# DakeQQ/Automatic-Speech-Recognition-ASR-ONNX

Measured on AMD Instinct MI355X. Metric: audio-sec/s, SenseVoiceSmall, 8 s @ 16 kHz chunks, batch 64 per GPU (RTF = 1/value per GPU-stream), higher is better.
Workload: dtype bf16; 1 GPU; SenseVoiceSmall bf16 (234 M params, 70 SANM blocks), batch=64 x 8 s per GPU, greedy CTC; step k's audio is resident in HBM when the step starts, batch k+1's host->device copy (pinned, copy stream) and every token-id download are inside the timed region; global_batch=64, parallelism=dp1 (utterance sharding, RCCL arena broadcast + hypothesis gather)

## Files before the change

automatic-speech-recognition-asr-onnx_amd/csrc/kernels.h:

```cpp
#pragma once
#include "common.h"

struct UttPlan {
  int64_t audio_off;
  int32_t n_samples;
  int32_t n_frames;
  int32_t frame_off;
  int32_t n_lfr;
  int32_t T;
  int32_t row_off;
  int32_t lang;
  int32_t blk0;
};

enum { AUDIO_F32 = 0, AUDIO_I16 = 1, AUDIO_F16 = 2 };
inline size_t audio_elt_bytes(int audio_dtype) { return audio_dtype == AUDIO_F32 ? 4 : 2; }
struct FbankArgs {
  const void* audio;
  const UttPlan* plan;
  const int32_t* blk_utt;
  const int32_t* blk_f0;
  const float* dft_packed;
  const float* mel_packed;
  float* mel_out;
// ... 51 lines not shown
template <typename T>
void launch_decode_attention(const DecAttnArgs& a, int batch, hipStream_t s);
const char* decode_attn_last_kernel();

constexpr int BEAM_MAX = 8;
void launch_beam_topk(const float* logits, int ld, int rows, int n_valid, const float* bias, int K, float* topv, int32_t* topi, hipStream_t s);
struct BeamArgs {
  int beam, K, ld, first, n_slots;
  const float* topv; const int32_t* topi;
  float* cum; int32_t* fin; int32_t* len; int32_t* next; int32_t* done;
  const int32_t* stop; int n_stop;
  const int32_t *src_in, *tok_in; int32_t *src_out, *tok_out;
  const int32_t* slots_dev = nullptr;
  int slots_off = 0;
};
void launch_beam_select(const BeamArgs& a, int n_utt, hipStream_t s);

void launch_argmax_rows(const float* logits, int ld, int rows, int n_valid, const float* extra, int32_t* ids, hipStream_t s);
void launch_no_speech_prob(const float* logits, int ld, int rows, int n_valid, const float* penalty, int no_speech_id, float* prob, hipStream_t s);

void launch_apply_penalty(float* logits, int ld, int rows, const int32_t* save_ids, int ld_save, const int32_t* n_saved,
                          int range, float value, hipStream_t s, int partial = 0);
void launch_append_ids(const int32_t* next, int rows, int32_t* save_ids, int ld_save, const int32_t* n_saved, hipStream_t s);

struct SampleArgs {
  float* logits; int ld; int rows; int n_valid;
  const float* extra;
  const int32_t* save_ids; int ld_save; const int32_t* n_saved;
  float temperature, top_p, repetition_penalty; int top_k;
  const float* noise; uint64_t seed;
  int32_t* next;
};
void launch_sample_topk_topp(const SampleArgs& a, hipStream_t s);

struct LfrArgs {
  const float* mel;
  const UttPlan* plan;
  const int32_t* row_utt;
  const float* cmvn_means;
  const float* cmvn_vars;
  const float* speech_pos;
  const float* language_embed;
  const float* system_embed;
  float* out;
  int ld_out, feat, n_mels, lfr_m, lfr_n, n_prompt, n_rows;
  int affine_mode = 0;
  bf16_t* out_lo = nullptr;
};
void launch_lfr_cmvn(const LfrArgs& a, hipStream_t s);

template <typename OutT>
void launch_layernorm(const float* x, int ld_x, int rows, int D, const float* gamma, const float* beta, float eps,
                      OutT* out, int ld_out, int fill_to, hipStream_t s, const int32_t* rows_dev = nullptr);


struct AttnArgs {
  const void* q; const void* k; int ld_qk;
  int ld_q = 0;
  const void* vt; int ld_vt;
  void* ctx; int ld_ctx;
  const UttPlan* plan;
  const int32_t* qb_utt;
  const int32_t* qb_q0;
  int n_qblocks, n_heads;
  int qt = 0, n_waves = 4, max_T = 0;
  const UttPlan* q_plan = nullptr;
  int causal = 0, kv_group = 1;
};
void attention_geometry(int max_T, int head_dim, int* qt, int* n_waves);
void launch_attention_bf16_hd128(const AttnArgs& a, hipStream_t s);
void launch_attention_bf16_hd64(const AttnArgs& a, hipStream_t s);
void launch_attention_f32(const AttnArgs& a, int head_dim, hipStream_t s);

struct SanmFusedArgs {
  const void* h; int ld_h; int K;
  const void* wqkv; int ldw;
  const float* bqkv;
  const float* wfsmn; const float* bfsmn;
  const UttPlan* plan; int n_utts, n_heads, d;
  void* ctx; int ld_ctx;
  float* mem; int ld_mem;
  int n_rows_alloc;
  const float* ln_colsum = nullptr; int ln_dim = 0; float ln_eps = 1e-5f;
  const float2* ln_stats_in = nullptr; int ln_slots = 0;
  int dbg = 0;
};
bool sanm_fused_supported(int max_T, int d_head, int n_heads, int d, int fsmn_taps, int K);

struct SanmBlockLayer {
  const float *bqkv, *cqkv, *wfsmn, *bfsmn, *b1, *c1, *b2;
  const void* wpack;
};
struct SanmBlockArgs {
  const bf16_t* wqkv; const float* bqkv; const float* cqkv;
  const float* wfsmn; const float* bfsmn;
  const bf16_t* wout;
  const bf16_t* w1; const float* b1; const float* c1;
  const bf16_t* w2; const float* b2;
  const SanmBlockLayer* layers = nullptr; int n_layers = 1;
  int flag_stride = 0;
  unsigned* place = nullptr;
  int times_layer = 0;
  int st_in_n = 16;
  int opt = 0;
  int ffnk = 0;
  const void* wpack = nullptr;
// ... 144 lines not shown
```

automatic-speech-recognition-asr-onnx_amd/csrc/kernels.hip:

```cpp
#include "kernels.h"
#include "gemm.h"

#include <algorithm>
#include <type_traits>
#include <cstdlib>

namespace {

constexpr int HOP = 160, WIN = 400;
constexpr int FB_FRAMES = 64;
constexpr int FB_SPAN = (FB_FRAMES - 1) * HOP + WIN;
constexpr int FB_AUDIO_LDS = FB_SPAN + FB_SPAN / HOP + 16;
constexpr int FB_PLD = 273;

template <typename S> struct Pcm;
template <> struct Pcm<float> {
  typedef float raw_t;
  static __device__ __forceinline__ raw_t load(const float* p, int i) { return p[i]; }
  static __device__ __forceinline__ raw_t hold(raw_t r) { return r; }
  static __device__ __forceinline__ float widen(raw_t r, float) { return r; }
};
template <> struct Pcm<int16_t> {
  typedef int raw_t;
  static __device__ __forceinline__ raw_t load(const int16_t* p, int i) { return p[i]; }
// ... 293 lines not shown
    const int k = kc * 32 + fgrp * 8 + e;
    float v = 0.0f;
    if (k < n_kchunks16 * 16) {
      v = dft_packed[(((size_t)tr * n_kchunks16 + (k >> 4)) * 64 + ((k & 3) * 16 + frow)) * 4 + ((k & 15) >> 2)];
    }
    float r = v;
    for (int z = 0; z < 3; ++z) {
      const uint32_t b = pack_bf16x2(r, 0.0f) & 0xffffu;
      r -= __uint_as_float(b << 16);
      w[z][e >> 1] |= b << ((e & 1) * 16);
    }
  }
  for (int z = 0; z < 3; ++z) out[((size_t)(tr * FB_K32 + kc) * 3 + z) * 64 + lane] = make_uint4(w[z][0], w[z][1], w[z][2], w[z][3]);
}

__global__ void lfr_cmvn_kernel(const LfrArgs a) {
  const int m = blockIdx.x;
  float* o = a.out + (size_t)m * a.ld_out;
  const int u = a.row_utt[m];
  bf16_t* olo = a.out_lo ? a.out_lo + (size_t)m * a.ld_out : nullptr;
  if (u < 0) {
    for (int c = threadIdx.x; c < a.ld_out; c += blockDim.x) { o[c] = 0.0f; if (olo) olo[c] = 0; }
    return;
  }
  const UttPlan up = a.plan[u];
  const int t = m - up.row_off;
  const int left = (a.lfr_m - 1) / 2;
  for (int c = threadIdx.x; c < a.ld_out; c += blockDim.x) {
    float v = 0.0f;
    if (c < a.feat && t < up.T) {
      if (a.n_prompt > 0 && t == 0) {
        v = a.language_embed[(size_t)up.lang * a.feat + c];
      } else if (t < a.n_prompt) {
        v = a.system_embed[(size_t)(t - 1) * a.feat + c];
      } else {
        const int j = t - a.n_prompt;
        int f = j * a.lfr_n + c / a.n_mels - left;
        f = min(max(f, 0), up.n_frames - 1);
        const float x = a.mel[(size_t)(up.frame_off + f) * a.n_mels + c % a.n_mels];
        if (a.affine_mode == 1) {
          v = x * a.cmvn_vars[c] + a.speech_pos[(size_t)j * a.feat + c];
        } else {
          v = (x + a.cmvn_means[c]) * a.cmvn_vars[c];
          v = v + a.speech_pos[(size_t)j * a.feat + c];
        }
      }
    }
    o[c] = v;
    if (olo) olo[c] = f32_to_bf16(v);
  }
}

constexpr int LN_MAXV = 8;
template <typename OutT>
__global__ __launch_bounds__(256) void layernorm_kernel(const float* __restrict__ x, int ld_x, int rows, int D,
                                                        const float* __restrict__ gamma, const float* __restrict__ beta,
                                                        float eps, OutT* out, int ld_out, int fill_to, const int32_t* __restrict__ rows_dev) {
  const int row = blockIdx.x * 4 + (threadIdx.x >> 6);
  const int lane = threadIdx.x & 63;
  if (row >= rows || (rows_dev && row >= *rows_dev)) return;
  const float* xr = x + (size_t)row * ld_x;
  float4 v[LN_MAXV];
  float s = 0.0f;
#pragma unroll
  for (int k = 0; k < LN_MAXV; ++k) {
    const int i = k * 256 + lane * 4;
    v[k] = (i < D) ? *reinterpret_cast<const float4*>(xr + i) : make_float4(0.f, 0.f, 0.f, 0.f);
    s += (v[k].x + v[k].y) + (v[k].z + v[k].w);
  }
  const float mean = wave_sum(s) / (float)D;
  float q = 0.0f;
#pragma unroll
  for (int k = 0; k < LN_MAXV; ++k) {
    const int i = k * 256 + lane * 4;
    if (i < D) {
      const float a = v[k].x - mean, b = v[k].y - mean, c = v[k].z - mean, d = v[k].w - mean;
      q += (a * a + b * b) + (c * c + d * d);
    }
  }
  const float var = wave_sum(q) / (float)D;
  const float rstd = 1.0f / sqrtf(var + eps);
  OutT* o = out + (size_t)row * ld_out;
#pragma unroll
  for (int k = 0; k < LN_MAXV; ++k) {
    const int i = k * 256 + lane * 4;
    if (i < D) {
      float y0 = (v[k].x - mean) * rstd, y1 = (v[k].y - mean) * rstd, y2 = (v[k].z - mean) * rstd, y3 = (v[k].w - mean) * rstd;
      if (gamma) {
        const float4 g = *reinterpret_cast<const float4*>(gamma + i);
        const float4 b = *reinterpret_cast<const float4*>(beta + i);
        y0 = y0 * g.x + b.x; y1 = y1 * g.y + b.y; y2 = y2 * g.z + b.z; y3 = y3 * g.w + b.w;
      }
      if constexpr (sizeof(OutT) == 4) {
        *reinterpret_cast<float4*>(o + i) = make_float4(y0, y1, y2, y3);
      } else {
        uint2 w;
        w.x = pack_bf16x2(y0, y1);
        w.y = pack_bf16x2(y2, y3);
        *reinterpret_cast<uint2*>(o + i) = w;
      }
    }
  }
  for (int i = D + lane; i < fill_to; i += 64) Elem<OutT>::store(o + i, 0.0f);
}

__global__ __launch_bounds__(256) void layernorm_fp8_kernel(const float* __restrict__ x, int ld_x, int rows, int D, float eps, float inv_scale,
                                                            unsigned char* __restrict__ out, int ld_out) {
  const int row = blockIdx.x * 4 + (threadIdx.x >> 6), lane = threadIdx.x & 63;
  if (row >= rows) return;
  const float* xr = x + (size_t)row * ld_x;
  float4 v[8];
  const int nv = D >> 8;
  float s1 = 0.0f;
#pragma unroll
  for (int k = 0; k < 8; ++k)
    if (k < nv) { v[k] = *reinterpret_cast<const float4*>(xr + k * 256 + lane * 4); s1 += (v[k].x + v[k].y) + (v[k].z + v[k].w); }
  const float mean = wave_sum(s1) / (float)D;
  float s2 = 0.0f;
#pragma unroll
  for (int k = 0; k < 8; ++k)
    if (k < nv) { const float a = v[k].x - mean, b = v[k].y - mean, c = v[k].z - mean, d = v[k].w - mean; s2 += (a * a + b * b) + (c * c + d * d); }
  const float rstd = rsqrtf(wave_sum(s2) / (float)D + eps) * inv_scale;
#pragma unroll
  for (int k = 0; k < 8; ++k)
    if (k < nv) {
      auto q = [&](float t) { return fminf(fmaxf((t - mean) * rstd, -448.0f), 448.0f); };
      int w = 0;
      w = __builtin_amdgcn_cvt_pk_fp8_f32(q(v[k].x), q(v[k].y), w, false);
      w = __builtin_amdgcn_cvt_pk_fp8_f32(q(v[k].z), q(v[k].w), w, true);
      *reinterpret_cast<int*>(out + (size_t)row * ld_out + k * 256 + lane * 4) = w;
    }
}

__device__ __forceinline__ float vmax3(float a, float b, float c) { return fmaxf(fmaxf(a, b), c); }

template <int HD, int CHUNK, int QT>
__global__ __launch_bounds__(512, (HD * QT <= 128) ? 4 : (HD * QT <= 256 ? 2 : 1)) void attn_bf16_kernel(const AttnArgs a, int n_rows_alloc) {
  constexpr int SLOTS = HD / 8;
  constexpr int KROWB = HD * 2;
  constexpr int K_RPI = 64 / SLOTS;
  constexpr int VSLOTS = CHUNK / 8;
  constexpr int VROWB = CHUNK * 2;
  constexpr int V_RPI = 64 / VSLOTS;
  constexpr int V_NI = HD / V_RPI;
  static_assert(VSLOTS == 16 || VSLOTS == 32, "V^T swizzle assumes 16 or 32 slots per row");
  extern __shared__ __attribute__((aligned(16))) unsigned char smem[];
  unsigned char* Ks = smem;
  unsigned char* Vs = smem + CHUNK * KROWB;

  const int tid = threadIdx.x, lane = tid & 63;
  const int wave = __builtin_amdgcn_readfirstlane(tid >> 6), NW = blockDim.x >> 6;
  const int fq = lane & 15, g = lane >> 4;
  const int u = a.qb_utt[blockIdx.x], q_base = a.qb_q0[blockIdx.x], h = blockIdx.y;
// ... 926 lines not shown
  ASR_REQUIRE(a.n_kchunks * 16 == WIN, "fbank: k-chunks must cover the window");
  const size_t lds = (size_t)(FB_AUDIO_LDS + FB_FRAMES * FB_PLD) * sizeof(float);
  static PerDeviceOnce attr_once;
  if (attr_once.first()) {
    HIP_CHECK(hipFuncSetAttribute(reinterpret_cast<const void*>(fbank_kernel<S>), hipFuncAttributeMaxDynamicSharedMemorySize, (int)lds));
  }
  if (a.dft_split) {
    FbankArgs b = a;
    if (const char* e = getenv("ASR_FBANK_DBG")) b.dbg = atoi(e);
    const size_t lds2 = (size_t)FB_A16 * 2 * 2 + (size_t)FB_FRAMES * FB_PLD * sizeof(float);
    static PerDeviceOnce attr2_once;
    if (attr2_once.first()) {
      HIP_CHECK(hipFuncSetAttribute(reinterpret_cast<const void*>(fbank_split_kernel<S>), hipFuncAttributeMaxDynamicSharedMemorySize, (int)lds2));
    }
    hipLaunchKernelGGL(fbank_split_kernel<S>, dim3(n_blocks), dim3(64 * FB_WAVES), lds2, s, b);
    HIP_CHECK(hipGetLastError());
    return;
  }
  hipLaunchKernelGGL(fbank_kernel<S>, dim3(n_blocks), dim3(256), lds, s, a);
  HIP_CHECK(hipGetLastError());
}
void launch_fbank(const FbankArgs& a, int n_blocks, hipStream_t s) {
  switch (a.audio_dtype) {
    case AUDIO_F32: return launch_fbank_typed<float>(a, n_blocks, s);
    case AUDIO_I16: return launch_fbank_typed<int16_t>(a, n_blocks, s);
    case AUDIO_F16: return launch_fbank_typed<_Float16>(a, n_blocks, s);
    default: ASR_THROW(ASR_ERR_INVALID, "fbank: unknown audio sample type %d", a.audio_dtype);
  }
}

size_t fbank_split_table_bytes(int n_bin_tiles, int win) {
  ASR_REQUIRE(win == WIN, "fbank: only win=400 is built (got %d)", win);
  return (size_t)n_bin_tiles * 2 * FB_K32 * 3 * 64 * 16;
}
void launch_fbank_split_table(const float* dft_packed, int n_bin_tiles, int n_kchunks16, void* out, hipStream_t s) {
  const int total = n_bin_tiles * 2 * FB_K32 * 64;
  hipLaunchKernelGGL(fbank_split_table_kernel, dim3((total + 255) / 256), dim3(256), 0, s, dft_packed, n_bin_tiles, n_kchunks16, reinterpret_cast<uint4*>(out));
  HIP_CHECK(hipGetLastError());
}

void launch_lfr_cmvn(const LfrArgs& a, hipStream_t s) {
  hipLaunchKernelGGL(lfr_cmvn_kernel, dim3(a.n_rows), dim3(256), 0, s, a);
  HIP_CHECK(hipGetLastError());
}

template <typename OutT>
void launch_layernorm(const float* x, int ld_x, int rows, int D, const float* gamma, const float* beta, float eps,
                      OutT* out, int ld_out, int fill_to, hipStream_t s, const int32_t* rows_dev) {
  ASR_REQUIRE(D % 4 == 0 && D <= LN_MAXV * 256 && ld_x % 4 == 0 && ld_out % 4 == 0, "layernorm: D=%d ld=%d unsupported", D, ld_x);
  hipLaunchKernelGGL(layernorm_kernel<OutT>, dim3((rows + 3) / 4), dim3(256), 0, s, x, ld_x, rows, D, gamma, beta, eps, out,
                     ld_out, fill_to, rows_dev);
  HIP_CHECK(hipGetLastError());
}
template void launch_layernorm<float>(const float*, int, int, int, const float*, const float*, float, float*, int, int, hipStream_t, const int32_t*);
template void launch_layernorm<bf16_t>(const float*, int, int, int, const float*, const float*, float, bf16_t*, int, int, hipStream_t, const int32_t*);

void launch_layernorm_fp8(const float* x, int ld_x, int rows, int D, float eps, float inv_scale, unsigned char* out, int ld_out, hipStream_t s) {
  ASR_REQUIRE(D % 256 == 0 && D <= 2048 && ld_x % 4 == 0 && ld_out % 4 == 0, "layernorm_fp8: D=%d unsupported", D);
  hipLaunchKernelGGL(layernorm_fp8_kernel, dim3((rows + 3) / 4), dim3(256), 0, s, x, ld_x, rows, D, eps, inv_scale, out, ld_out);
  HIP_CHECK(hipGetLastError());
}

template <int HD, int CHUNK, int QT>
static void launch_attn_inst(const AttnArgs& a, hipStream_t s) {
  constexpr int lds = CHUNK * HD * 2 * 2;
  static PerDeviceOnce attr_once;
  if (attr_once.first()) {
    HIP_CHECK(hipFuncSetAttribute(reinterpret_cast<const void*>(attn_bf16_kernel<HD, CHUNK, QT>),
                                  hipFuncAttributeMaxDynamicSharedMemorySize, lds));
  }
  AttnArgs b = a;
  if (b.ld_q == 0) b.ld_q = b.ld_qk;
  hipLaunchKernelGGL((attn_bf16_kernel<HD, CHUNK, QT>), dim3(a.n_qblocks, a.n_heads), dim3(64 * a.n_waves), lds, s, b, a.ld_vt);
  HIP_CHECK(hipGetLastError());
}

void attention_geometry(int max_T, int head_dim, int* qt, int* nw) {
  const int qt_max = 2;
  const int n_tiles = (max_T + 15) / 16;
  int q = 1;
  while (q < qt_max && (n_tiles + q - 1) / q > 8) ++q;
  if (const char* e = getenv("ASR_ATTN_QT")) q = std::max(1, std::min(qt_max, atoi(e)));
  int w = std::min(8, (n_tiles + q - 1) / q);
  if (const char* e = getenv("ASR_ATTN_NW")) w = std::max(1, std::min(8, atoi(e)));
  *qt = q;
  *nw = w;
}

void launch_attention_bf16_hd128(const AttnArgs& a, hipStream_t s) {
  ASR_REQUIRE(a.qt >= 1 && a.qt <= 2 && a.n_waves >= 1 && a.n_waves <= 8, "attention: bad geometry qt=%d nw=%d", a.qt, a.n_waves);
  const bool big = a.max_T <= 256;
  if (a.qt == 1) { big ? launch_attn_inst<128, 256, 1>(a, s) : launch_attn_inst<128, 128, 1>(a, s); }
  else { big ? launch_attn_inst<128, 256, 2>(a, s) : launch_attn_inst<128, 128, 2>(a, s); }
}
void launch_attention_bf16_hd64(const AttnArgs& a, hipStream_t s) {
  ASR_REQUIRE(a.qt >= 1 && a.qt <= 2 && a.n_waves >= 1 && a.n_waves <= 8, "attention: bad geometry qt=%d nw=%d", a.qt, a.n_waves);
  if (a.qt == 1) launch_attn_inst<64, 256, 1>(a, s); else launch_attn_inst<64, 256, 2>(a, s);
}

void launch_attention_f32(const AttnArgs& a, int head_dim, hipStream_t s) {
  ASR_REQUIRE(head_dim <= 128 && head_dim % 4 == 0, "attention_f32: head_dim %d unsupported", head_dim);
  AttnArgs b = a;
  if (b.ld_q == 0) b.ld_q = b.ld_qk;
  const int wgs = a.n_qblocks * a.n_heads;
  const int z = wgs >= 1024 ? 1 : wgs >= 256 ? 4 : 16;
  hipLaunchKernelGGL(attn_f32_kernel, dim3(a.n_qblocks, a.n_heads, z), dim3(256), 0, s, b, head_dim);
// ... 1078 lines not shown
```

automatic-speech-recognition-asr-onnx_amd/csrc/sanm_block8.hip:

```cpp
#include <algorithm>
#include <type_traits>
#include <utility>
#include "kernels.h"

namespace {

constexpr int R = 144, RF = 9;
constexpr int HD = 128, NH = 4, D = 512, DFF = 2048;
constexpr int NW = 8, NT = NW * 64;
constexpr int TAPS = 11;
constexpr int LDS_BYTES = 160 * 1024;
constexpr int CH = R * 256;
constexpr int NSLOT = 4;
constexpr int QS = 0, KS = CH, KEYS = 160, VS = KS + KEYS * 256, IMG_END = VS + HD * 512;
constexpr int TERM = CH;
constexpr int RED = 2 * CH;
constexpr int ST_F = NSLOT * CH;
constexpr int ST_P = ST_F + R * 8;
constexpr int DUMMY = ST_P + NSLOT * R * 8;
static_assert(IMG_END <= ST_F && TERM + R * HD * 4 <= ST_F && DUMMY + NW * 256 <= LDS_BYTES, "LDS map");

constexpr size_t PK_QKV = 0, PK_QKV_WAVE = 16 * 3 * 1024;
constexpr size_t PK_OUT = PK_QKV + (size_t)NH * NW * PK_QKV_WAVE, PK_OUT_WAVE = 8 * 2 * 1024;
constexpr size_t PK_W1 = PK_OUT + (size_t)NH * NW * PK_OUT_WAVE, PK_W1_WAVE = 16 * 4 * 1024;
constexpr size_t PK_W2 = PK_W1 + (size_t)NH * NW * PK_W1_WAVE, PK_W2_WAVE = 32 * 2 * 1024;
constexpr size_t PK_BYTES = PK_W2 + (size_t)NH * NW * PK_W2_WAVE;
static_assert(PK_BYTES == (size_t)(3 * D * D + D * D + 2 * DFF * D) * 2, "the packed copy holds every weight element once");

__device__ __host__ constexpr int frag_col(int j, int fr) { return (j >> 1) * 32 + ((fr >> 2) << 3) + ((j & 1) << 2) + (fr & 3); }
template <int N> __device__ __forceinline__ void wait_vm() { asm volatile("s_waitcnt vmcnt(%0)" ::"n"(N) : "memory"); }

typedef __attribute__((ext_vector_type(4))) unsigned int u32x4_t;
__device__ __forceinline__ void store16_wt(void* p, uint4 v, bool plain = false) {
  if (plain) { *reinterpret_cast<uint4*>(p) = v; return; }
  const u32x4_t w = {v.x, v.y, v.z, v.w};
  asm volatile("global_store_dwordx4 %0, %1, off sc1\n\ts_nop 1" ::"v"(p), "v"(w) : "memory");
}
__device__ __forceinline__ void store8_wt(void* p, float2 v, bool plain = false) {
  if (plain) { *reinterpret_cast<float2*>(p) = v; return; }
  const f32x2_t w = {v.x, v.y};
  asm volatile("global_store_dwordx2 %0, %1, off sc1\n\ts_nop 1" ::"v"(p), "v"(w) : "memory");
}

__device__ __forceinline__ void publish(unsigned* flag, bool withhold = false) {
  wait_vm<0>();
  __syncthreads();
  if (threadIdx.x == 0 && !withhold) __hip_atomic_fetch_add(flag, 1u, __ATOMIC_RELAXED, __HIP_MEMORY_SCOPE_AGENT);
}
__device__ __forceinline__ void consume(unsigned* flag, unsigned need, unsigned* err, bool fence = true) {
  if (threadIdx.x == 0) {
    unsigned spins = 0;
    while (__hip_atomic_load(flag, __ATOMIC_RELAXED, __HIP_MEMORY_SCOPE_AGENT) < need) {
      __builtin_amdgcn_s_sleep(2);
      if (++spins > (1u << 15)) { __hip_atomic_store(err, 1u, __ATOMIC_RELAXED, __HIP_MEMORY_SCOPE_AGENT); break; }
      if ((spins & 255u) == 0u && __hip_atomic_load(err, __ATOMIC_RELAXED, __HIP_MEMORY_SCOPE_AGENT)) break;
    }
    if (fence) __builtin_amdgcn_fence(__ATOMIC_ACQUIRE, "agent");
  }
  __syncthreads();
}

__device__ __forceinline__ uint4 pack8(const float (&v)[8]) {
  uint4 w;
  w.x = pack_bf16x2(v[0], v[1]); w.y = pack_bf16x2(v[2], v[3]); w.z = pack_bf16x2(v[4], v[5]); w.w = pack_bf16x2(v[6], v[7]);
  return w;
}
__device__ __forceinline__ void stats8(const uint4& w, float& s1, float& s2) {
  const uint32_t wd[4] = {w.x, w.y, w.z, w.w};
#pragma unroll
  for (int e = 0; e < 4; ++e) {
    const float lo = __uint_as_float(wd[e] << 16), hi = __uint_as_float(wd[e] & 0xffff0000u);
    s1 += lo + hi;
    s2 = fmaf(lo, lo, fmaf(hi, hi, s2));
// ... 347 lines not shown
          const float2 ss = sum_row_partials(a->st_in + (size_t)(row0 + min(tid, rows_left - 1)) * (D / 32), D / 32);
          const float mean = ss.x * (1.0f / D);
          const float var = fmaxf(ss.y * (1.0f / D) - mean * mean, 0.0f);
          st_fin[tid] = make_float2(mean, rsqrtf(var + a->ln_eps));
        }
        __syncthreads();
      } else row_stats_from_chunks(smem, h, a->ln_eps, tid);
      STAMP_A(4);
      {
        unsigned char* dst = smem + (grp == 0 ? QS : KS);
        const float b8[8] = {b0.x, b0.y, b0.z, b0.w, b1.x, b1.y, b1.z, b1.w}, c8[8] = {c0.x, c0.y, c0.z, c0.w, c1.x, c1.y, c1.z, c1.w};
#pragma unroll
        for (int i = 0; i < RF; ++i) {
          const int row = i * 16 + frow;
          const float2 mr = st_fin[row];
          float v[8];
#pragma unroll
          for (int r = 0; r < 4; ++r) { v[r] = acc[i][0][r]; v[4 + r] = acc[i][1][r]; }
#pragma unroll
          for (int e = 0; e < 8; ++e) v[e] = (v[e] - mr.x * c8[e]) * mr.y + b8[e];
          *reinterpret_cast<uint4*>(dst + row * 256 + ((((col >> 3)) ^ (row & 15)) << 4)) = pack8(v);
        }
        unsigned char* vdst = smem + VS + dcol * 512 + (fgrp & 1) * 8;
#pragma unroll
        for (int i = 0; i < RF; ++i) {
          float v[4] = {acc[i][2][0], acc[i][2][1], acc[i][2][2], acc[i][2][3]};
#pragma unroll
          for (int r = 0; r < 4; ++r) { const float2 mr = st_fin[i * 16 + fgrp * 4 + r]; v[r] = (v[r] - mr.x * cs) * mr.y + bv; }
          uint2 w;
          w.x = pack_bf16x2(v[0], v[1]);
          w.y = pack_bf16x2(v[2], v[3]);
          *reinterpret_cast<uint2*>(vdst + (((2 * i + (fgrp >> 1)) ^ (dcol & 15)) << 4)) = w;
        }
        if (tid < 2 * HD) {
          const int d = tid & (HD - 1), slot = 18 + (tid >> 7);
          *reinterpret_cast<uint4*>(smem + VS + d * 512 + ((slot ^ (d & 15)) << 4)) = make_uint4(0, 0, 0, 0);
        }
      }
    }
    __syncthreads();
    STAMP_A(5);
    float wc[TAPS];
#pragma unroll
    for (int j = 0; j < TAPS; ++j) wc[j] = L->wfsmn[(h * HD + (tid & (HD - 1))) * TAPS + j];
    const float bc = L->bfsmn[h * HD + (tid & (HD - 1))];

    {
      const unsigned char* Qs = smem + QS;
      const unsigned char* Ks = smem + KS;
      const unsigned char* Vs = smem + VS;
      const int fq = frow, g = fgrp;
      const int n_sub = (T + 31) >> 5;
      const bool shared_tile = T > 128;
      auto scores = [&](const bf16x8_t (&qf)[HD / 32], bf16x8_t (&pf)[5], float& inv) {
        constexpr float LOG2E = 1.4426950408889634f;
        f32x4_t st[5][2];
#pragma unroll
        for (int s = 0; s < 5; ++s) { st[s][0] = f32x4_t{0.f, 0.f, 0.f, 0.f}; st[s][1] = f32x4_t{0.f, 0.f, 0.f, 0.f}; }
#pragma unroll
        for (int s = 0; s < 5; ++s) {
          if (s < n_sub) {
            const int key0 = s * 32 + ((fq >> 2) << 3) + (fq & 3), key1 = key0 + 4;
#pragma unroll
            for (int ks = 0; ks < HD / 32; ++ks) {
              const int c = ks * 4 + g;
              const bf16x8_t kf0 = *reinterpret_cast<const bf16x8_t*>(Ks + key0 * 256 + ((c ^ (key0 & 15)) << 4));
              const bf16x8_t kf1 = *reinterpret_cast<const bf16x8_t*>(Ks + key1 * 256 + ((c ^ (key1 & 15)) << 4));
              st[s][0] = __builtin_amdgcn_mfma_f32_16x16x32_bf16(kf0, qf[ks], st[s][0], 0, 0, 0);
              st[s][1] = __builtin_amdgcn_mfma_f32_16x16x32_bf16(kf1, qf[ks], st[s][1], 0, 0, 0);
            }
          }
        }
        float mx = -INFINITY;
#pragma unroll
        for (int s = 0; s < 5; ++s) {
          if (s * 32 + 32 > T) {
#pragma unroll
            for (int hlf = 0; hlf < 2; ++hlf)
#pragma unroll
              for (int r = 0; r < 4; ++r)
                if (s * 32 + g * 8 + hlf * 4 + r >= T) st[s][hlf][r] = -INFINITY;
          }
          mx = fmaxf(fmaxf(fmaxf(mx, fmaxf(st[s][0][0], st[s][0][1])), fmaxf(st[s][0][2], st[s][0][3])), fmaxf(fmaxf(st[s][1][0], st[s][1][1]), fmaxf(st[s][1][2], st[s][1][3])));
        }
        mx = fmaxf(mx, __shfl_xor(mx, 16, 64));
        mx = fmaxf(mx, __shfl_xor(mx, 32, 64));
        const f32x2_t mneg = {-mx * LOG2E, -mx * LOG2E}, l2 = {LOG2E, LOG2E};
        f32x2_t lsum = {0.0f, 0.0f};
#pragma unroll
        for (int s = 0; s < 5; ++s) {
          f32x2_t p[4];
#pragma unroll
          for (int q = 0; q < 4; ++q) {
            const f32x2_t e = __builtin_elementwise_fma(f32x2_t{st[s][q >> 1][2 * (q & 1)], st[s][q >> 1][2 * (q & 1) + 1]}, l2, mneg);
            p[q] = f32x2_t{__builtin_amdgcn_exp2f(e[0]), __builtin_amdgcn_exp2f(e[1])};
          }
          lsum += (p[0] + p[1]) + (p[2] + p[3]);
          union { bf16x8_t v; uint32_t w[4]; } u8;
#pragma unroll
          for (int q = 0; q < 4; ++q) u8.w[q] = pack_bf16x2(p[q][0], p[q][1]);
          pf[s] = u8.v;
        }
        float l = lsum[0] + lsum[1];
        l += __shfl_xor(l, 16, 64);
        l += __shfl_xor(l, 32, 64);
        inv = 1.0f / l;
      };
      auto context = [&](const bf16x8_t (&pf)[5], float inv, int qrow, auto dt0_tag, auto nd_tag) {
        constexpr int ND = decltype(nd_tag)::value;
        const int dt0 = dt0_tag;
        f32x4_t ot[ND];
#pragma unroll
        for (int e = 0; e < ND; ++e) ot[e] = f32x4_t{0.f, 0.f, 0.f, 0.f};
#pragma unroll
        for (int s = 0; s < 5; ++s) {
          if (s < n_sub) {
#pragma unroll
            for (int e = 0; e < ND; ++e) {
              const int d = (dt0 + e) * 16 + fq;
              const bf16x8_t vf = *reinterpret_cast<const bf16x8_t*>(Vs + d * 512 + (((s * 4 + g) ^ (d & 15)) << 4));
              ot[e] = __builtin_amdgcn_mfma_f32_16x16x32_bf16(vf, pf[s], ot[e], 0, 0, 0);
            }
          }
        }
        unsigned char* crow = smem + QS + qrow * 256;
#pragma unroll
        for (int e = 0; e < ND; ++e) {
          uint2 w;
          w.x = pack_bf16x2(ot[e][0] * inv, ot[e][1] * inv);
          w.y = pack_bf16x2(ot[e][2] * inv, ot[e][3] * inv);
          *reinterpret_cast<uint2*>(crow + ((((dt0 + e) * 2 + (g >> 1)) ^ (qrow & 15)) << 4) + (g & 1) * 8) = w;
        }
      };
      if (wave * 16 < T) {
        const int qrow = wave * 16 + fq;
        bf16x8_t qf[HD / 32], pf[5];
#pragma unroll
        for (int ks = 0; ks < HD / 32; ++ks) qf[ks] = *reinterpret_cast<const bf16x8_t*>(Qs + qrow * 256 + (((ks * 4 + g) ^ (qrow & 15)) << 4));
        float inv;
        scores(qf, pf, inv);
        context(pf, inv, qrow, 0, std::integral_constant<int, HD / 16>{});
      }
      STAMP_A(6);
      if (shared_tile) {
        bf16x8_t qf8[HD / 32], pf[5];
        const int qrow8 = 128 + fq;
#pragma unroll
        for (int ks = 0; ks < HD / 32; ++ks) qf8[ks] = *reinterpret_cast<const bf16x8_t*>(Qs + qrow8 * 256 + (((ks * 4 + g) ^ (qrow8 & 15)) << 4));
        float inv;
        scores(qf8, pf, inv);
        __syncthreads();
        context(pf, inv, 128 + fq, wave, std::integral_constant<int, 1>{});
      }
      STAMP_A(7);
    }
    __syncthreads();
    STAMP(2);
    {
      const bool plain = cluster_plain_stores(place, a->opt);
      if (a->times && tid == 0) a->times[(size_t)blockIdx.x * 16 + 15] = plain ? 1ull : 0ull;
      const int T16 = n_act * 16;
      for (int c = T * 16 + tid; c < T16 * 16; c += NT) *reinterpret_cast<uint4*>(smem + QS + c * 16) = make_uint4(0, 0, 0, 0);
      __syncthreads();
      store_chunk_img(reinterpret_cast<unsigned char*>(a->ctx + (size_t)row0 * D) + (size_t)h * T16 * 256, smem + QS, n_act * 4, wave, lane, plain);
    }
    STAMP(3);
#pragma unroll
    for (int i = 0; i < RF; ++i) {
      if (kh == 0) {
        const float* xr = a->x + (size_t)(row0 + min(i * 16 + frow, rows_left - 1)) * D + h * HD + cg * 32 + fgrp * 8;
        accb[i][0] = *reinterpret_cast<const f32x4_t*>(xr); accb[i][1] = *reinterpret_cast<const f32x4_t*>(xr + 4);
      } else { accb[i][0] = f32x4_t{0.f, 0.f, 0.f, 0.f}; accb[i][1] = f32x4_t{0.f, 0.f, 0.f, 0.f}; }
    }
    {
      constexpr int PAD = (TAPS - 1) / 2;
      const int c = tid & (HD - 1), seg = tid >> 7;
      const int t0 = seg < 2 ? seg * 40 : 80 + (seg - 2) * 32, len = seg < 2 ? 40 : 32;
      const unsigned char* vrow = smem + VS + c * 512;
      float x[56];
#pragma unroll
      for (int q = 0; q < 7; ++q) {
        const int sl = (t0 >> 3) - 1 + q;
        if (sl < 0 || sl * 8 >= T) {
#pragma unroll
          for (int e = 0; e < 8; ++e) x[q * 8 + e] = 0.0f;
        } else {
          const uint4 raw = *reinterpret_cast<const uint4*>(vrow + ((sl ^ (c & 15)) << 4));
          const uint32_t wds[4] = {raw.x, raw.y, raw.z, raw.w};
#pragma unroll
          for (int e = 0; e < 4; ++e) {
            x[q * 8 + 2 * e] = (sl * 8 + 2 * e < T) ? __uint_as_float(wds[e] << 16) : 0.0f;
            x[q * 8 + 2 * e + 1] = (sl * 8 + 2 * e + 1 < T) ? __uint_as_float(wds[e] & 0xffff0000u) : 0.0f;
          }
        }
      }
      float y[40];
#pragma unroll
      for (int i = 0; i < 40; ++i) {
        float accv = bc;
#pragma unroll
        for (int j = 0; j < TAPS; ++j) accv = fmaf(wc[j], x[8 + i + j - PAD], accv);
        y[i] = accv;
      }
// ... 419 lines not shown
```

automatic-speech-recognition-asr-onnx_amd/csrc/sensevoice.hip:

```cpp
#include <cstdlib>
#include <cstring>
#include <type_traits>

#include "../../include/asr_mi355x.h"
#include "engine.h"
#include "gemm.h"
#include "kernels.h"

namespace {

struct SvBlock {
  const float *ln1_g, *ln1_b, *bqkv, *wfsmn, *bfsmn, *ln2_g, *ln2_b, *b1, *b2;
  const float *cqkv, *c1;
  const void *wqkv, *wout, *w1, *w2;
  int in_size, kpad;
};

inline int round_up(int v, int m) { return (v + m - 1) / m * m; }

struct SvRunCtx;

struct PfDecLayer {
  const void *w1, *w2, *wq, *wkv, *wo;
  const float *b1, *b2, *n2_g, *n2_b, *wfsmn, *bq, *bkv, *bo;
// ... 327 lines not shown
  const bool tiles = r.tiles && block_cooldown == 0 && !foreign_now;
  HIP_CHECK(hipMemsetAsync(d_flags.ptr, 0, (tile_flag0 + (tiles ? (size_t)c.n_blocks * tile_flag_stride : 0)) * 4, stream));
  const float* x_in = d_x0.as<float>();
  const bf16_t* x_in_lo = x0lo;
  const float2* st_in = nullptr;
  bool st_in_block8 = false;
  float2* sta = d_sta.as<float2>();
  float2* stb = d_stb.as<float2>();
  int ld_in = kpad0;
  float* xa = d_xa.as<float>();
  float* xb = d_xb.as<float>();
  T* h = d_h.as<T>();
  T* qk = d_qk.as<T>();
  T* vt = d_vt.as<T>();
  T* ctx = d_ctx.as<T>();
  float* mem = d_mem.as<float>();
  T* ffn = d_ffn.as<T>();
  for (int i = 0; i < c.n_blocks; ++i) {
    const SvBlock& b = blocks[i];
    if constexpr (sizeof(T) == 2) {
      if (blk && b.in_size == d && x_in == xa) {
        if (!alg && i == 1) {
          ProfScope ps0(prof, "layernorm", stream);
          launch_rows_to_bf16(xa, xalo, (size_t)Mpad * d, stream);
          st_in = nullptr;
        }
        const int per = sanm_block_max_utts();
        const int run_end = (!paraformer && i < c.n_main) ? c.n_main : c.n_blocks;
        const int n_run = block_persist ? run_end - i : 1;
        for (int u0 = 0; u0 < r.batch; u0 += per) {
          ProfScope ps(prof, "sanm_block", stream);
          SanmBlockArgs ba{};
          ba.wqkv = (const bf16_t*)b.wqkv; ba.bqkv = b.bqkv; ba.cqkv = b.cqkv; ba.wfsmn = b.wfsmn; ba.bfsmn = b.bfsmn;
          ba.wout = (const bf16_t*)b.wout; ba.w1 = (const bf16_t*)b.w1; ba.b1 = b.b1; ba.c1 = b.c1; ba.w2 = (const bf16_t*)b.w2; ba.b2 = b.b2;
          ba.x_lo = xalo; ba.st_in = st_in; ba.x = xa; ba.x_lo_out = xalo; ba.st_out = sta;
          ba.ctx = (bf16_t*)ctx; ba.x1_lo = xblo; ba.st1 = stb; ba.hid = (bf16_t*)ffn;
          ba.plan = r.dp; ba.utt0 = u0; ba.n_utts = std::min(per, r.batch - u0);
          ba.flags = d_flags.as<unsigned>() + ((size_t)i * r.batch + u0) * 4; ba.err = d_flags.as<unsigned>() + flag_words;
          ba.flag_stride = r.batch * 4; ba.place = d_flags.as<unsigned>() + flag_words + 4 + (size_t)i * r.batch + u0;
          ba.n_rows_alloc = Mpad; ba.ln_eps = 1e-5f; ba.scatter = block_scatter; ba.fault = (block_fault && i == 1) ? 1 : 0;
          if (block_dbg >= i && block_dbg < i + n_run && u0 == 0) {
            d_times.reserve(256 * 16 * 8, stream); HIP_CHECK(hipMemsetAsync(d_times.ptr, 0, 256 * 16 * 8, stream)); ba.times = d_times.as<unsigned long long>();
            ba.times_layer = block_dbg - i;
          }
          ba.layers = d_layer_tab.as<SanmBlockLayer>() + i; ba.n_layers = n_run; ba.opt = block8_opt; ba.ffnk = block_ffnk ? 1 : 0;
          ba.st_in_n = st_in_block8 ? 4 : 16;
          launch_sanm_block8(ba, stream);
        }
        i += n_run - 1;
        st_in = sta;
        st_in_block8 = true;
        if (i == c.n_main - 1 && !paraformer) {
          ProfScope ps2(prof, "layernorm", stream);
          launch_layernorm<bf16_t>(xa, d, rows, d, after_g, after_b, 1e-5f, xalo, d, d, stream); st_in = nullptr;
          launch_layernorm<float>(xa, d, rows, d, after_g, after_b, 1e-5f, xa, d, d, stream);
        }
        continue;
      }
    }
    if constexpr (sizeof(T) == 2) {
      if (tiles && !blk && b.in_size == d && x_in == xa) {
        const int run_end = (!paraformer && i < c.n_main) ? c.n_main : c.n_blocks;
        {
          ProfScope ps(prof, "sanm_tiles", stream);
          SanmTilesArgs ta;
          ta.plan = r.dp; ta.tile_win = r.d_tile_win; ta.tile_idx = r.d_tile_idx; ta.n_tiles = r.n_tiles; ta.n_windows = r.batch; ta.n_layers = run_end - i;
          ta.ln_eps = 1e-5f; ta.layers = d_tlayer_tab.as<StreamLayer>() + i;
          ta.x = xa; ta.xb = xb; ta.ctx = (bf16_t*)ctx; ta.hid = (bf16_t*)ffn; ta.kv = d_tkv.as<bf16_t>(); ta.kv_parity_stride = (size_t)Mpad * 2 * d;
          ta.flags = d_flags.as<unsigned>() + tile_flag0 + (size_t)i * tile_flag_stride; ta.flag_stride = (int)tile_flag_stride;
          ta.err = d_flags.as<unsigned>() + flag_words; ta.opt = tiles_opt;
          if (tiles_dbg >= i && tiles_dbg < run_end) {
            d_times.reserve(256 * 16 * 8, stream); HIP_CHECK(hipMemsetAsync(d_times.ptr, 0, 256 * 16 * 8, stream)); ta.times = d_times.as<unsigned long long>();
            ta.times_layer = tiles_dbg - i;
          }
          launch_sanm_tiles(ta, stream);
        }
        i = run_end - 1;
        st_in = nullptr;
        if (i == c.n_main - 1 && !paraformer) {
          ProfScope ps2(prof, "layernorm", stream);
          launch_layernorm<float>(xa, d, rows, d, after_g, after_b, 1e-5f, xa, d, d, stream);
        }
        continue;
      }
    }
    if (!alg) {
      ProfScope ps(prof, "layernorm", stream);
      launch_layernorm<T>(x_in, ld_in, rows, b.in_size, b.ln1_g, b.ln1_b, 1e-5f, h, b.kpad, b.kpad, stream);
    }
    const bool fused = use_fused && precision == ASR_PRECISION_BF16 &&
                       sanm_fused_supported(r.max_T, c.d_head, c.n_heads, d, c.fsmn_kernel, b.kpad);
    if (fused) {
      ProfScope ps(prof, "sanm_fused", stream);
      SanmFusedArgs fa;
      fa.h = h; fa.ld_h = b.kpad; fa.K = b.kpad;
      if (alg) { fa.h = x_in_lo; fa.ln_colsum = b.cqkv; fa.ln_dim = b.in_size; fa.ln_stats_in = st_in; fa.ln_slots = d / 32; } fa.wqkv = b.wqkv; fa.ldw = b.kpad; fa.bqkv = b.bqkv;
      fa.wfsmn = b.wfsmn; fa.bfsmn = b.bfsmn; fa.plan = r.dp; fa.n_utts = r.batch; fa.n_heads = c.n_heads; fa.d = d;
      fa.ctx = ctx; fa.ld_ctx = d; fa.mem = mem; fa.ld_mem = d; fa.n_rows_alloc = Mpad;
      launch_sanm_qkv_attn(fa, stream);
    } else {
      {
        ProfScope ps(prof, "gemm_qkv", stream);
        GemmArgs g;
        g.A = h; g.lda = b.kpad; g.W = b.wqkv; g.ldw = b.kpad; g.M = rows; g.N = 2 * d; g.K = b.kpad; g.bias = b.bqkv;
        g.out_lo = qk; g.ld_out_lo = 2 * d;
        gemm(g);
        GemmArgs gv;
        gv.A = h; gv.lda = b.kpad; gv.W = (const T*)b.wqkv + (size_t)2 * d * b.kpad; gv.ldw = b.kpad; gv.M = rows; gv.N = d;
// ... 1 lines not shown
        gemm(gv);
      }
      {
        ProfScope ps(prof, "fsmn", stream);
        launch_fsmn<T>(vt, Mpad, b.wfsmn, b.bfsmn, d, c.fsmn_kernel, r.dp, r.d_row_utt, Mpad, mem, d, stream);
      }
      {
        ProfScope ps(prof, "attention", stream);
        AttnArgs aa;
        aa.q = qk; aa.k = qk + d; aa.ld_qk = 2 * d; aa.vt = vt; aa.ld_vt = Mpad; aa.ctx = ctx; aa.ld_ctx = d;
        aa.plan = r.dp; aa.qb_utt = r.d_qb_utt; aa.qb_q0 = r.d_qb_q0; aa.n_qblocks = r.n_qb; aa.n_heads = c.n_heads;
        aa.qt = r.att_qt; aa.n_waves = r.att_nw; aa.max_T = r.max_T;
        if (precision == ASR_PRECISION_BF16) launch_attention_bf16_hd128(aa, stream);
        else launch_attention_f32(aa, c.d_head, stream);
      }
    }
    {
      ProfScope ps(prof, "gemm_out", stream);
      GemmArgs g;
      g.A = ctx; g.lda = d; g.W = b.wout; g.ldw = d; g.M = rows; g.N = d; g.K = d;
      g.add = mem; g.ld_add = d;
      if (b.in_size == d) { g.add2 = x_in; g.ld_add2 = ld_in; }
      g.out_f32 = xb; g.ld_out_f32 = d;
      if (alg) { g.out_lo = xblo; g.ld_out_lo = d; g.st_out = stb; }
      gemm(g);
    }
    if (!alg) {
      ProfScope ps(prof, "layernorm", stream);
      launch_layernorm<T>(xb, d, rows, d, b.ln2_g, b.ln2_b, 1e-5f, h, d, d, stream);
    }
    {
      ProfScope ps(prof, "gemm_ffn1", stream);
      GemmArgs g;
      g.A = h; g.lda = d; g.W = b.w1; g.ldw = d; g.M = rows; g.N = dff; g.K = d; g.bias = b.b1; g.act = ACT_RELU;
      g.out_lo = ffn; g.ld_out_lo = dff;
      if (alg) { g.A = xblo; g.ln_colsum = b.c1; g.ln_dim = d; g.ln_stats_in = stb; g.ln_slots = d / 32; }
      gemm(g);
    }
    {
      ProfScope ps(prof, "gemm_ffn2", stream);
      GemmArgs g;
      g.A = ffn; g.lda = dff; g.W = b.w2; g.ldw = dff; g.M = rows; g.N = d; g.K = dff; g.bias = b.b2;
      g.add = xb; g.ld_add = d; g.out_f32 = xa; g.ld_out_f32 = d;
      if (alg) { g.out_lo = xalo; g.ld_out_lo = d; g.st_out = sta; }
      gemm(g);
    }
    x_in = xa;
    x_in_lo = xalo;
    st_in = sta;
    ld_in = d;
    if (i == 0) save_tap("block0", xa, rows, d, d, 4);
    if (i == c.n_main - 1 && !paraformer) {
      ProfScope ps(prof, "layernorm", stream);
      if (alg) { launch_layernorm<bf16_t>(xa, d, rows, d, after_g, after_b, 1e-5f, xalo, d, d, stream); st_in = nullptr; }
      launch_layernorm<float>(xa, d, rows, d, after_g, after_b, 1e-5f, xa, d, d, stream);
    }
  }
  if (paraformer) { copy_block_status(r); enqueue_paraformer_tail<T>(r); return; }
  if (taps_enabled) {
    launch_layernorm<float>(xa, d, rows, d, tp_g, tp_b, 1e-5f, xb, d, d, stream);
    save_tap("enc_out", xb, rows, d, d, 4);
  }
  {
    ProfScope ps(prof, "layernorm", stream);
    launch_layernorm<T>(xa, d, rows, d, tp_g, tp_b, 1e-5f, h, d, d, stream);
  }
  {
    ProfScope ps(prof, "gemm_ctc", stream);
    GemmArgs g;
    g.A = h; g.lda = d; g.W = ctc_w; g.ldw = d; g.M = rows; g.N = vpad; g.K = d; g.bias = ctc_b;
    g.amax_val = d_amax_v.as<float>(); g.amax_idx = d_amax_i.as<int32_t>(); g.n_valid = c.vocab;
    if (taps_enabled) { g.out_f32 = d_logits.as<float>(); g.ld_out_f32 = vpad; }
    gemm(g);
  }
  {
    ProfScope ps(prof, "ctc_tail", stream);
    launch_argmax_reduce(d_amax_v.as<float>(), d_amax_i.as<int32_t>(), rows, n_slabs, d_ids.as<int32_t>(), stream);
    launch_ctc_collapse(d_ids.as<int32_t>(), r.dp, r.batch, c.blank_id, d_tok.as<int32_t>(), r.max_tokens, d_num.as<int32_t>(), stream);
  }
  if (taps_enabled) {
    save_tap("logits", d_logits.ptr, rows, c.vocab, vpad, 4);
    save_tap("frame_ids", d_ids.ptr, rows, 1, 1, 4);
  }
  HIP_CHECK(hipMemcpyAsync(h_out.ptr, d_tok.ptr, (size_t)r.batch * r.max_tokens * 4, hipMemcpyDeviceToHost, stream));
  HIP_CHECK(hipMemcpyAsync(h_out.as<unsigned char>() + (size_t)r.batch * r.max_tokens * 4, d_num.ptr, (size_t)r.batch * 4,
                           hipMemcpyDeviceToHost, stream));
  copy_block_status(r);
}


template <typename T>
void SvSession::enqueue_paraformer_tail(const SvRunCtx& r) {
  const auto& c = cfg;
  const int d = c.d_model, dd = pcfg.d_dec_ffn, rows = r.rows, Mpad = r.Mpad, n_slabs = vpad / 64;
  float* xa = d_xa.as<float>();
  float* enc32 = d_xb.as<float>();
  T* enc_lo = d_enc_lo.as<T>();
  T* h = d_h.as<T>();
  T* q = d_qk.as<T>();
  T* ck = d_ck.as<T>();
  T* cvt = d_vt.as<T>();
  T* ctx = d_ctx.as<T>();
  T* ffn = d_ffn.as<T>();
  float* ffn32 = d_ffn32.as<float>();
  float* x1 = d_mem.as<float>();
  float* dec = d_dec.as<float>();
  float* x2 = d_x2.as<float>();
  float* x2_own = d_sa.as<float>();
// ... 985 lines not shown
```

Measured before the change: 79020 audio-s/s.

## Compute ninth query tile scores once across waves and fuse dual layernorm

In the SANM block8 attention path, when T exceeds 128 the ninth 16-row query tile was scored redundantly by every wave. Now waves 0-4 each compute one key sub-tile of those scores, reusing the K fragments already loaded for their own rows. They hand the partial maxima, probabilities and row sums over through new LDS regions with two extra barriers, so the other waves no longer repeat the full score pass. Separately, the post-encoder layernorm writes bf16 and fp32 outputs from one kernel instead of two launches. This removes a re-read of the activations and one launch, though the kernel now writes its fp32 result in place over its own input.

```diff
diff --git a/automatic-speech-recognition-asr-onnx_amd/csrc/kernels.h b/automatic-speech-recognition-asr-onnx_amd/csrc/kernels.h
--- a/automatic-speech-recognition-asr-onnx_amd/csrc/kernels.h
+++ b/automatic-speech-recognition-asr-onnx_amd/csrc/kernels.h
@@ -127,6 +127,7 @@
 template <typename OutT>
 void launch_layernorm(const float* x, int ld_x, int rows, int D, const float* gamma, const float* beta, float eps,
                       OutT* out, int ld_out, int fill_to, hipStream_t s, const int32_t* rows_dev = nullptr);
+void launch_layernorm_dual(const float* x, int ld_x, int rows, int D, const float* gamma, const float* beta, float eps, bf16_t* out_lo, float* out_f, int ld_out, hipStream_t s);
 
 
 struct AttnArgs {
diff --git a/automatic-speech-recognition-asr-onnx_amd/csrc/kernels.hip b/automatic-speech-recognition-asr-onnx_amd/csrc/kernels.hip
--- a/automatic-speech-recognition-asr-onnx_amd/csrc/kernels.hip
+++ b/automatic-speech-recognition-asr-onnx_amd/csrc/kernels.hip
@@ -369,10 +369,10 @@
 }
 
 constexpr int LN_MAXV = 8;
-template <typename OutT>
+template <typename OutT, bool DUAL = false>
 __global__ __launch_bounds__(256) void layernorm_kernel(const float* __restrict__ x, int ld_x, int rows, int D,
                                                         const float* __restrict__ gamma, const float* __restrict__ beta,
-                                                        float eps, OutT* out, int ld_out, int fill_to, const int32_t* __restrict__ rows_dev) {
+                                                        float eps, OutT* out, int ld_out, int fill_to, const int32_t* __restrict__ rows_dev, float* out_f = nullptr) {
   const int row = blockIdx.x * 4 + (threadIdx.x >> 6);
   const int lane = threadIdx.x & 63;
   if (row >= rows || (rows_dev && row >= *rows_dev)) return;
@@ -416,6 +416,7 @@
         w.y = pack_bf16x2(y2, y3);
         *reinterpret_cast<uint2*>(o + i) = w;
       }
+      if constexpr (DUAL) *reinterpret_cast<float4*>(out_f + (size_t)row * ld_out + i) = make_float4(y0, y1, y2, y3);
     }
   }
   for (int i = D + lane; i < fill_to; i += 64) Elem<OutT>::store(o + i, 0.0f);
@@ -1448,6 +1449,12 @@
                      ld_out, fill_to, rows_dev);
   HIP_CHECK(hipGetLastError());
 }
+void launch_layernorm_dual(const float* x, int ld_x, int rows, int D, const float* gamma, const float* beta, float eps, bf16_t* out_lo, float* out_f, int ld_out, hipStream_t s) {
+  ASR_REQUIRE(D % 4 == 0 && D <= LN_MAXV * 256 && ld_x % 4 == 0 && ld_out % 4 == 0, "layernorm: D=%d ld=%d unsupported", D, ld_x);
+  hipLaunchKernelGGL((layernorm_kernel<bf16_t, true>), dim3((rows + 3) / 4), dim3(256), 0, s, x, ld_x, rows, D, gamma, beta, eps, out_lo,
+                     ld_out, D, (const int32_t*)nullptr, out_f);
+  HIP_CHECK(hipGetLastError());
+}
 template void launch_layernorm<float>(const float*, int, int, int, const float*, const float*, float, float*, int, int, hipStream_t, const int32_t*);
 template void launch_layernorm<bf16_t>(const float*, int, int, int, const float*, const float*, float, bf16_t*, int, int, hipStream_t, const int32_t*);
 
diff --git a/automatic-speech-recognition-asr-onnx_amd/csrc/sanm_block8.hip b/automatic-speech-recognition-asr-onnx_amd/csrc/sanm_block8.hip
--- a/automatic-speech-recognition-asr-onnx_amd/csrc/sanm_block8.hip
+++ b/automatic-speech-recognition-asr-onnx_amd/csrc/sanm_block8.hip
@@ -18,7 +18,11 @@
 constexpr int ST_F = NSLOT * CH;
 constexpr int ST_P = ST_F + R * 8;
 constexpr int DUMMY = ST_P + NSLOT * R * 8;
+constexpr int T8_MX = DUMMY + NW * 256;
+constexpr int T8_P = T8_MX + 512;
+constexpr int T8_T = T8_P + 5 * 1024;
 static_assert(IMG_END <= ST_F && TERM + R * HD * 4 <= ST_F && DUMMY + NW * 256 <= LDS_BYTES, "LDS map");
+static_assert(5 * 16 * 4 <= T8_P - T8_MX && T8_P % 16 == 0 && T8_T % 8 == 0 && T8_T + 5 * 512 <= LDS_BYTES, "LDS map: ninth-tile hand-over");
 
 constexpr size_t PK_QKV = 0, PK_QKV_WAVE = 16 * 3 * 1024;
 constexpr size_t PK_OUT = PK_QKV + (size_t)NH * NW * PK_QKV_WAVE, PK_OUT_WAVE = 8 * 2 * 1024;
@@ -472,8 +476,10 @@
       const int fq = frow, g = fgrp;
       const int n_sub = (T + 31) >> 5;
       const bool shared_tile = T > 128;
-      auto scores = [&](const bf16x8_t (&qf)[HD / 32], bf16x8_t (&pf)[5], float& inv) {
-        constexpr float LOG2E = 1.4426950408889634f;
+      const bool once8 = shared_tile && !(a->opt & 1024);
+      const bool score8 = once8 && wave < 5;
+      constexpr float LOG2E = 1.4426950408889634f;
+      auto scores = [&](const bf16x8_t (&qf)[HD / 32], bf16x8_t (&pf)[5], float& inv, bool x8, const bf16x8_t (&qf8)[HD / 32], f32x4_t (&st8)[2]) {
         f32x4_t st[5][2];
 #pragma unroll
         for (int s = 0; s < 5; ++s) { st[s][0] = f32x4_t{0.f, 0.f, 0.f, 0.f}; st[s][1] = f32x4_t{0.f, 0.f, 0.f, 0.f}; }
@@ -481,13 +487,21 @@
         for (int s = 0; s < 5; ++s) {
           if (s < n_sub) {
             const int key0 = s * 32 + ((fq >> 2) << 3) + (fq & 3), key1 = key0 + 4;
+            bf16x8_t kf0[HD / 32], kf1[HD / 32];
 #pragma unroll
             for (int ks = 0; ks < HD / 32; ++ks) {
               const int c = ks * 4 + g;
-              const bf16x8_t kf0 = *reinterpret_cast<const bf16x8_t*>(Ks + key0 * 256 + ((c ^ (key0 & 15)) << 4));
-              const bf16x8_t kf1 = *reinterpret_cast<const bf16x8_t*>(Ks + key1 * 256 + ((c ^ (key1 & 15)) << 4));
-              st[s][0] = __builtin_amdgcn_mfma_f32_16x16x32_bf16(kf0, qf[ks], st[s][0], 0, 0, 0);
-              st[s][1] = __builtin_amdgcn_mfma_f32_16x16x32_bf16(kf1, qf[ks], st[s][1], 0, 0, 0);
+              kf0[ks] = *reinterpret_cast<const bf16x8_t*>(Ks + key0 * 256 + ((c ^ (key0 & 15)) << 4));
+              kf1[ks] = *reinterpret_cast<const bf16x8_t*>(Ks + key1 * 256 + ((c ^ (key1 & 15)) << 4));
+              st[s][0] = __builtin_amdgcn_mfma_f32_16x16x32_bf16(kf0[ks], qf[ks], st[s][0], 0, 0, 0);
+              st[s][1] = __builtin_amdgcn_mfma_f32_16x16x32_bf16(kf1[ks], qf[ks], st[s][1], 0, 0, 0);
+            }
+            if (x8 && s == wave) {
+#pragma unroll
+              for (int ks = 0; ks < HD / 32; ++ks) {
+                st8[0] = __builtin_amdgcn_mfma_f32_16x16x32_bf16(kf0[ks], qf8[ks], st8[0], 0, 0, 0);
+                st8[1] = __builtin_amdgcn_mfma_f32_16x16x32_bf16(kf1[ks], qf8[ks], st8[1], 0, 0, 0);
+              }
             }
           }
         }
@@ -552,23 +566,71 @@
           *reinterpret_cast<uint2*>(crow + ((((dt0 + e) * 2 + (g >> 1)) ^ (qrow & 15)) << 4) + (g & 1) * 8) = w;
         }
       };
+      f32x4_t st8[2] = {f32x4_t{0.f, 0.f, 0.f, 0.f}, f32x4_t{0.f, 0.f, 0.f, 0.f}};
       if (wave * 16 < T) {
         const int qrow = wave * 16 + fq;
-        bf16x8_t qf[HD / 32], pf[5];
+        bf16x8_t qf[HD / 32], qf8[HD / 32], pf[5];
 #pragma unroll
         for (int ks = 0; ks < HD / 32; ++ks) qf[ks] = *reinterpret_cast<const bf16x8_t*>(Qs + qrow * 256 + (((ks * 4 + g) ^ (qrow & 15)) << 4));
+        const int qrow8 = score8 ? 128 + fq : qrow;
+#pragma unroll
+        for (int ks = 0; ks < HD / 32; ++ks) qf8[ks] = score8 ? *reinterpret_cast<const bf16x8_t*>(Qs + qrow8 * 256 + (((ks * 4 + g) ^ (qrow8 & 15)) << 4)) : qf[ks];
         float inv;
-        scores(qf, pf, inv);
+        scores(qf, pf, inv, score8, qf8, st8);
+        if (score8) {
+          const int s = wave;
+          if (s * 32 + 32 > T) {
+#pragma unroll
+            for (int hlf = 0; hlf < 2; ++hlf)
+#pragma unroll
+              for (int r = 0; r < 4; ++r)
+                if (s * 32 + g * 8 + hlf * 4 + r >= T) st8[hlf][r] = -INFINITY;
+          }
+          float m8 = fmaxf(fmaxf(fmaxf(st8[0][0], st8[0][1]), fmaxf(st8[0][2], st8[0][3])), fmaxf(fmaxf(st8[1][0], st8[1][1]), fmaxf(st8[1][2], st8[1][3])));
+          m8 = fmaxf(m8, __shfl_xor(m8, 16, 64));
+          m8 = fmaxf(m8, __shfl_xor(m8, 32, 64));
+          if (g == 0) reinterpret_cast<float*>(smem + T8_MX)[s * 16 + fq] = m8;
+        }
         context(pf, inv, qrow, 0, std::integral_constant<int, HD / 16>{});
       }
       STAMP_A(6);
-      if (shared_tile) {
+      if (once8) {
+        __syncthreads();
+        if (score8) {
+          const float* m5 = reinterpret_cast<const float*>(smem + T8_MX) + fq;
+          float mx = -INFINITY;
+#pragma unroll
+          for (int s = 0; s < 5; ++s) mx = fmaxf(mx, m5[s * 16]);
+          const f32x2_t mneg = {-mx * LOG2E, -mx * LOG2E}, l2 = {LOG2E, LOG2E};
+          f32x2_t p[4];
+#pragma unroll
+          for (int q = 0; q < 4; ++q) {
+            const f32x2_t e = __builtin_elementwise_fma(f32x2_t{st8[q >> 1][2 * (q & 1)], st8[q >> 1][2 * (q & 1) + 1]}, l2, mneg);
+            p[q] = f32x2_t{__builtin_amdgcn_exp2f(e[0]), __builtin_amdgcn_exp2f(e[1])};
+          }
+          const f32x2_t ts = (p[0] + p[1]) + (p[2] + p[3]);
+          *reinterpret_cast<uint4*>(smem + T8_P + wave * 1024 + lane * 16) = make_uint4(pack_bf16x2(p[0][0], p[0][1]), pack_bf16x2(p[1][0], p[1][1]), pack_bf16x2(p[2][0], p[2][1]), pack_bf16x2(p[3][0], p[3][1]));
+          *reinterpret_cast<f32x2_t*>(smem + T8_T + wave * 512 + lane * 8) = ts;
+        }
+        __syncthreads();
+        bf16x8_t pf[5];
+#pragma unroll
+        for (int s = 0; s < 5; ++s) pf[s] = *reinterpret_cast<const bf16x8_t*>(smem + T8_P + s * 1024 + lane * 16);
+        f32x2_t lsum = *reinterpret_cast<const f32x2_t*>(smem + T8_T + lane * 8);
+#pragma unroll
+        for (int s = 1; s < 5; ++s) lsum += *reinterpret_cast<const f32x2_t*>(smem + T8_T + s * 512 + lane * 8);
+        float l = lsum[0] + lsum[1];
+        l += __shfl_xor(l, 16, 64);
+        l += __shfl_xor(l, 32, 64);
+        context(pf, 1.0f / l, 128 + fq, wave, std::integral_constant<int, 1>{});
+      } else if (shared_tile) {
         bf16x8_t qf8[HD / 32], pf[5];
         const int qrow8 = 128 + fq;
 #pragma unroll
         for (int ks = 0; ks < HD / 32; ++ks) qf8[ks] = *reinterpret_cast<const bf16x8_t*>(Qs + qrow8 * 256 + (((ks * 4 + g) ^ (qrow8 & 15)) << 4));
         float inv;
-        scores(qf8, pf, inv);
+        f32x4_t none[2];
+        scores(qf8, pf, inv, false, qf8, none);
         __syncthreads();
         context(pf, inv, 128 + fq, wave, std::integral_constant<int, 1>{});
       }
diff --git a/automatic-speech-recognition-asr-onnx_amd/csrc/sensevoice.hip b/automatic-speech-recognition-asr-onnx_amd/csrc/sensevoice.hip
--- a/automatic-speech-recognition-asr-onnx_amd/csrc/sensevoice.hip
+++ b/automatic-speech-recognition-asr-onnx_amd/csrc/sensevoice.hip
@@ -403,8 +403,7 @@
         st_in_block8 = true;
         if (i == c.n_main - 1 && !paraformer) {
           ProfScope ps2(prof, "layernorm", stream);
-          launch_layernorm<bf16_t>(xa, d, rows, d, after_g, after_b, 1e-5f, xalo, d, d, stream); st_in = nullptr;
-          launch_layernorm<float>(xa, d, rows, d, after_g, after_b, 1e-5f, xa, d, d, stream);
+          launch_layernorm_dual(xa, d, rows, d, after_g, after_b, 1e-5f, xalo, xa, d, stream); st_in = nullptr;
         }
         continue;
       }
@@ -512,8 +511,8 @@
     if (i == 0) save_tap("block0", xa, rows, d, d, 4);
     if (i == c.n_main - 1 && !paraformer) {
       ProfScope ps(prof, "layernorm", stream);
-      if (alg) { launch_layernorm<bf16_t>(xa, d, rows, d, after_g, after_b, 1e-5f, xalo, d, d, stream); st_in = nullptr; }
-      launch_layernorm<float>(xa, d, rows, d, after_g, after_b, 1e-5f, xa, d, d, stream);
+      if (alg) { launch_layernorm_dual(xa, d, rows, d, after_g, after_b, 1e-5f, xalo, xa, d, stream); st_in = nullptr; }
+      else launch_layernorm<float>(xa, d, rows, d, after_g, after_b, 1e-5f, xa, d, d, stream);
     }
   }
   if (paraformer) { copy_block_status(r); enqueue_paraformer_tail<T>(r); return; }
```

Result: no change. 79540 audio-s/s (median of 6 runs) (+0.7%).
